# rebots-online/InstantIR

Hardware: AMD Instinct MI355X
Metric: denoising steps/sec at 1024x1024 (InstantIR step: previewer UNet + LCM + Aggregator + UNet, CFG) (higher is better)
Workload: dtype f16 (fp32 accumulate); 1 GPU; BASELINE configs[1]: 1024x1024, batch 1/GPU, cfg 7.0 (2 rows), 30-step DDIM timetable, preview_start 0, full SDXL+TA-IP UNet x2 + Aggregator per step; images_per_gpu=1, weight_elements=4422072388, graph=True, finite=True, world=1

## Files before the change

### instantir_amd/csrc/gemm_conv.hip

```cpp
#include "common.h"
#include "gemm_geo.h"
#include "../../include/instantir_hip.h"
#include <stdlib.h>
#include <type_traits>

namespace {

using iir::Geo;

constexpr int BK = 64;
#define IIR_PIN() __builtin_amdgcn_sched_barrier(0)
constexpr int PF_TOUCHES = 4;

constexpr int gn_par(int bm, bool lw) { return lw && bm == 128 ? 2 : 1; }
constexpr int ring_bytes(int bm, int bn, int st, bool w8) { return st * (bm * 128 + (w8 ? bn * 64 : bn * 128)); }
constexpr int scratch_bytes(int waves_m, bool lw) { return 256 * waves_m * 2 * (lw ? 2 : 1); }
constexpr int lds_bytes(int bm, int bn, int st, int waves_m, bool w8, bool lw) { return ring_bytes(bm, bn, st, w8) + scratch_bytes(waves_m, lw) + bm * 8; }
constexpr int lnp_off(int bm, int bn) { return (bm * (2 * bn + 32) + 15) / 16 * 16; }
constexpr bool ln_out_fits(int bm, int bn, int st, bool w8) { return lnp_off(bm, bn) + bm * (bn / 8) * 8 <= ring_bytes(bm, bn, st, w8); }
constexpr bool gn_out_fits(int bm, int bn, int st, int nt, bool lw, bool w8 = false) {
    const int gnt = nt / gn_par(bm, lw);
    return bm % 64 == 0 && bn <= gnt && (long)lnp_off(bm, bn) + (long)gn_par(bm, lw) * (gnt / (bn / 8)) * bn * 8 <= ring_bytes(bm, bn, st, w8);
}

template <int N>
__device__ __forceinline__ void wait_vm_lgkm_and_barrier() {
    asm volatile("s_waitcnt vmcnt(%0) lgkmcnt(0)\n\ts_barrier" ::"n"(N) : "memory");
}

template <int N>
__device__ __forceinline__ void wait_vm_and_barrier() {
    asm volatile("s_waitcnt vmcnt(%0)\n\ts_barrier" ::"n"(N) : "memory");
}

template <typename E, int BM, int BN, int ST, bool CONV, int WAVES_M = 2, bool W8 = false, bool LW = false, bool F8 = false>
__global__ __launch_bounds__(128 * WAVES_M * (LW ? 2 : 1), (WAVES_M == 2 ? 2 : 1)) void gemm_kernel(const Geo g) {
    static_assert(!(F8 && (W8 || CONV)), "the all-fp8 build covers the linear layers; W8 is the fp16-activation form");
    static_assert(!(W8 && CONV), "the fp8-weight build covers the linear layers only");
    static_assert(!(LW && W8), "loader waves: fp16 / bf16 operands only");
    static_assert(ST >= 2 && ST <= 4, "ring depths the counted waits below cover");
    using E4 = typename ET<E>::x4;
    using E8 = typename ET<E>::x8;
    constexpr int NW = WAVES_M * 2;
    constexpr int NT = 64 * NW * (LW ? 2 : 1);
    constexpr int WM = BM / WAVES_M, WN = BN / 2;
    constexpr int MI = WM / 16, NI = WN / 16;
    constexpr int B_GROUPS = W8 ? BN / 16 : BN / 8;
    constexpr int A_INST = BM / 8 / NW, B_INST = (B_GROUPS + NW - 1) / NW;
    static_assert(W8 || B_GROUPS % NW == 0, "fp16 weight tile: every wave issues the same number of row groups");
    constexpr int B_STAGE_BYTES = W8 ? BN * 64 : BN * 128;
    constexpr int RING_BYTES = ring_bytes(BM, BN, ST, W8);
    extern __shared__ __attribute__((aligned(16))) char smem[];
    f16* As = (f16*)smem;
    f16* Bs = As + ST * BM * BK;
    constexpr int LOADS = A_INST + B_INST;
    constexpr int SCRATCH_BYTES = scratch_bytes(WAVES_M, LW);
    float2* rowstat = (float2*)(smem + RING_BYTES + SCRATCH_BYTES);
    constexpr int LNP_OFF = lnp_off(BM, BN);
    constexpr bool LN_OUT_FITS = ln_out_fits(BM, BN, ST, W8);
    constexpr int GN_PAR = gn_par(BM, LW), GN_NT = NT / GN_PAR;
    constexpr int GN_RG = GN_NT / (BN / 8);
    constexpr bool GN_OUT_FITS = gn_out_fits(BM, BN, ST, NT, LW, W8);

    const int tid = threadIdx.x;
    const int lane = tid & 63;
    const int wave_all = __builtin_amdgcn_readfirstlane(tid >> 6);
    const bool loader = LW && wave_all >= NW;
    const int wave = loader ? wave_all - NW : wave_all;
    const int wm = wave >> 1, wn = wave & 1;

    int tm, tn;
    if (!iir::tile_of_block(g, tm, tn)) return;
    const int m0 = tm * BM, n0 = tn * BN;

    const int srow = lane >> 3;
    const int schunk = (lane & 7) ^ srow;
    const f16* a_src[A_INST];
    int a_pix_y[A_INST], a_pix_x[A_INST];
    const f16* a_img[A_INST];
#pragma unroll
    for (int i = 0; i < A_INST; ++i) {
        int m = m0 + (i * NW + wave) * 8 + srow;
        if (m >= g.M) m = g.M - 1;
        if (!CONV) {
            a_src[i] = g.A + (long)m * g.lda + schunk * 8;
        } else {
            const int hw = g.Ho * g.Wo;
            const int img = m / hw, rem = m - img * hw;
            const int oy = rem / g.Wo, ox = rem - oy * g.Wo;
            a_img[i] = g.A + (long)img * g.x_img_stride + schunk * 8;
            a_pix_y[i] = oy * g.stride - g.pad;
            a_pix_x[i] = ox * g.stride - g.pad;
        }
    }
    const f16* b_src[B_INST];
#pragma unroll
    for (int i = 0; i < B_INST; ++i) {
        if (!W8) {
            int n = n0 + (i * NW + wave) * 8 + srow;
            if (n >= g.N) n = g.N - 1;
            b_src[i] = g.W + (long)n * g.K + schunk * 8;
        } else {
            const int r = (i * NW + wave) * 16 + (lane >> 2);
            int n = n0 + r;
            if (n >= g.N) n = g.N - 1;
            b_src[i] = (const f16*)((const char*)g.W + (long)n * g.K + (((lane & 3) ^ ((r >> 2) & 3)) * 16));
        }
    }

    const f16* cv_ptr[CONV ? A_INST : 1];
    int cv_inc[CONV ? A_INST : 1];
    int cv_c0 = 0, cv_tap = 0;
    auto conv_tap = [&](int tap) {
        const int ky = tap / g.ks, kx = tap - ky * g.ks;
#pragma unroll
        for (int i = 0; i < (CONV ? A_INST : 0); ++i) {
            const int iy = a_pix_y[i] + ky, ix = a_pix_x[i] + kx;
            bool ok;
            long pix;
// ... 60 lines not shown
        a_off[s] = (wm * WM + frow) * 128 + phys * 16;
        if (!W8) b_off[s] = (wn * WN + frow) * 128 + phys * 16;
        else b_off[s] = (wn * WN + frow) * 64 + ((((fq >> 1) + 2 * s) ^ ((frow >> 2) & 3)) * 16) + (fq & 1) * 8;
    }

    f32x4 acc[MI][NI];
#pragma unroll
    for (int i = 0; i < MI; ++i)
#pragma unroll
        for (int j = 0; j < NI; ++j) acc[i][j] = (f32x4){0.f, 0.f, 0.f, 0.f};

    const int nk = g.K / BK;
    if (!LW || loader) {
        if (CONV) conv_seek(0);
#pragma unroll
        for (int s = 0; s < ST - 1; ++s)
            if (s < nk) stage(s, s);
    }
    constexpr int MAXP = 8;
    float2 lnp_in[MAXP];
    const int ln_lt = LW ? tid - 64 * NW : tid;
    if (g.ln_in && ln_lt >= 0 && ln_lt < BM) {
        const int m = min(m0 + ln_lt, g.M - 1);
#pragma unroll
        for (int j = 0; j < MAXP; ++j)
            lnp_in[j] = ((const float2*)g.ln_in)[(long)min(j, g.ln_parts - 1) * g.M + m];

        float sm = 0.f;
#pragma unroll
        for (int j = 0; j < MAXP; ++j) sm += j < g.ln_parts ? lnp_in[j].x : 0.f;
        const float inv_p = 1.0f / (float)g.ln_parts, mean = sm * inv_p;
        float m2 = 0.f, dev = 0.f;
#pragma unroll
        for (int j = 0; j < MAXP; ++j) {
            const float d = lnp_in[j].x - mean;
            m2 += j < g.ln_parts ? lnp_in[j].y : 0.f;
            dev += j < g.ln_parts ? d * d : 0.f;
        }
        const float var = (m2 + (float)g.ln_part_cols * dev) * inv_p / (float)g.ln_part_cols;
        const float rstd = rsqrtf(var + g.ln_eps);
        rowstat[ln_lt] = make_float2(rstd, -rstd * mean);
        }

    using BF = std::conditional_t<W8, long, E8>;
    auto frags = [&](int buf, int s, E8 (&af)[MI], BF (&bf)[NI]) {
        const char* as = (const char*)(As + buf * BM * BK);
        const char* bs = (const char*)Bs + buf * B_STAGE_BYTES;
#pragma unroll
        for (int i = 0; i < MI; ++i) af[i] = *(const E8*)(as + a_off[s] + i * 16 * 128);
#pragma unroll
        for (int j = 0; j < NI; ++j) bf[j] = *(const BF*)(bs + b_off[s] + j * 16 * (W8 ? 64 : 128));
    };
    auto mma = [&](const E8 (&af)[MI], const BF (&bf)[NI]) {
        if constexpr (F8) {
#pragma unroll
            for (int i = 0; i < MI; ++i)
#pragma unroll
                for (int j = 0; j < NI; ++j)
                    acc[i][j] = iir::mfma16_f8x2(bf[j], af[i], acc[i][j]);
        } else if constexpr (!W8) {
#pragma unroll
            for (int i = 0; i < MI; ++i)
#pragma unroll
                for (int j = 0; j < NI; ++j)
                    acc[i][j] = ET<E>::mfma16(bf[j], af[i], acc[i][j]);
        } else {
            long a8[MI];
#pragma unroll
            for (int i = 0; i < MI; ++i) a8[i] = iir_fp8x8(af[i]);
#pragma unroll
            for (int i = 0; i < MI; ++i)
#pragma unroll
                for (int j = 0; j < NI; ++j)
                    acc[i][j] = __builtin_amdgcn_mfma_f32_16x16x32_fp8_fp8(bf[j], a8[i], acc[i][j], 0, 0, 0);
        }
    };
    auto admit = [&](int tiles_after) {
        if (ST >= 4 && tiles_after >= 2) wait_vm_lgkm_and_barrier<(ST >= 4 ? 2 * LOADS : 0)>();
        else if (ST >= 3 && tiles_after >= 1) wait_vm_lgkm_and_barrier<(ST >= 3 ? LOADS : 0)>();
        else wait_vm_lgkm_and_barrier<0>();
    };
    f32x4 pre_c1[NI];
    E4 pre_c0[NI];
    auto preload_cols = [&]() {
#pragma unroll
        for (int j = 0; j < NI; ++j) {
            const int nc = min(n0 + wn * WN + j * 16 + fq * 4, g.N - 4);
            pre_c1[j] = g.ln_in ? *(const f32x4*)(g.ln_colsum + nc) : (f32x4){0.f, 0.f, 0.f, 0.f};
            if (g.bias) pre_c0[j] = *(const E4*)((const E*)g.bias + nc);
            else for (int t = 0; t < 4; ++t) pre_c0[j][t] = (E)0.f;
        }
    };
    E8 a0[MI], a1[MI];
    BF b0[NI], b1[NI];
    auto admit2 = [&](int tiles_after) {
        __builtin_amdgcn_s_waitcnt(0xC07F);
        if (ST >= 4 && tiles_after >= 2) wait_vm_and_barrier<(ST >= 4 ? 2 * LOADS : 0)>();
        else if (ST >= 3 && tiles_after >= 1) wait_vm_and_barrier<(ST >= 3 ? LOADS : 0)>();
        else wait_vm_and_barrier<0>();
    };
    if constexpr (!LW) {
        {
            const int rem = nk - 1;
            admit(rem < ST - 2 ? rem : ST - 2);
            if (ST - 1 < nk) stage(ST - 1, ST - 1);
            frags(0, 0, a0, b0);
            IIR_PIN();
            frags(0, 1, a1, b1);
            IIR_PIN();
            mma(a0, b0);
        }
        int cur = 0;
        for (int kt = 1; kt < nk; ++kt) {
            const int rem = nk - 1 - kt;
            admit2(rem < ST - 2 ? rem : ST - 2);
            if (kt - 1 + ST < nk) stage(kt - 1 + ST, cur);
            cur = cur + 1 == ST ? 0 : cur + 1;
            frags(cur, 0, a0, b0);
            IIR_PIN();
            mma(a1, b1);
            frags(cur, 1, a1, b1);
            IIR_PIN();
            mma(a0, b0);
        }
        preload_cols();
        mma(a1, b1);
    } else if (loader) {
        {
            const int rem = nk - 1;
            admit(rem < ST - 2 ? rem : ST - 2);
            if (ST - 1 < nk) stage(ST - 1, ST - 1);
        }
        int cur = 0;
        for (int kt = 0; kt + 1 < nk; ++kt) {
            const int rem = nk - 2 - kt;
            admit(rem < ST - 2 ? rem : ST - 2);
            if (kt + ST < nk) stage(kt + ST, cur);
            cur = cur + 1 == ST ? 0 : cur + 1;
        }
    } else {
        admit(0);
        frags(0, 0, a0, b0);
        IIR_PIN();
        frags(0, 1, a1, b1);
        IIR_PIN();
        mma(a0, b0);
        int cur = 0;
        for (int kt = 1; kt < nk; ++kt) {
            admit2(0);
            cur = cur + 1 == ST ? 0 : cur + 1;
            frags(cur, 0, a0, b0);
            IIR_PIN();
            mma(a1, b1);
            frags(cur, 1, a1, b1);
            IIR_PIN();
            mma(a0, b0);
        }
        preload_cols();
        mma(a1, b1);
    }

    bool xdone = false;
    if constexpr (BM == 64 && BN == 128 && ST == 3 && !CONV && !W8 && !LW && WAVES_M == 2 && std::is_same<E, f16>::value) {
    if (g.xa_on) {
        constexpr int KROWS = 144, KIMG = KROWS * 128, VROW = 288, VIMG = 64 * VROW;
        static_assert(2 * KIMG + 2 * VIMG <= RING_BYTES, "K / V images of two heads must fit the idle ring");
        asm volatile("s_waitcnt lgkmcnt(0)\n\ts_barrier" ::: "memory");
        const int img = m0 / g.xa_tq, hd0 = n0 >> 6;
        char* kl = smem;
        char* vl = smem + 2 * KIMG;
        const int tk0 = g.xa_tk[0], tk1 = g.xa_tk[1];
        const int vch0 = (tk0 + 7) >> 3, vch1 = (tk1 + 7) >> 3;
#pragma unroll
        for (int it = 0; it < 9; ++it) {
            const int s = (it * 4 + wave) * 64 + lane, hh = s >= 1152 ? 1 : 0, sl = s - hh * 1152;
            const int row = sl >> 3, ch = (sl & 7) ^ (row & 7);
            const bool ip = row >= 80;
            const int key = ip ? min(row - 80, tk1 - 1) : min(row, tk0 - 1);
            const f16* src = (ip ? g.xa_k[1] + (long)img * g.xa_kb[1] + (long)key * g.xa_ldk[1]
                                 : g.xa_k[0] + (long)img * g.xa_kb[0] + (long)key * g.xa_ldk[0]) + (hd0 + hh) * 64 + ch * 8;
            glds16(src, kl + (it * 4 + wave) * 1024);
        }
#pragma unroll
        for (int it = 0; it < 9; ++it) {
            const int s = (it * 4 + wave) * 64 + lane, hh = s >= 1152 ? 1 : 0, sl = s - hh * 1152;
            const int d = sl / 18, c = sl - d * 18;
            const bool ip = c >= 10;
            const int cc = ip ? min(c - 10, vch1 - 1) : min(c, vch0 - 1);
            const long rowv = (long)((hd0 + hh) * 64 + d);
            const f16* src = (ip ? g.xa_vt[1] + rowv * g.xa_ldvt[1] + (long)img * g.xa_vb[1]
                                 : g.xa_vt[0] + rowv * g.xa_ldvt[0] + (long)img * g.xa_vb[0]) + cc * 8;
            glds16(src, vl + (it * 4 + wave) * 1024);
        }
        typedef E E4v __attribute__((ext_vector_type(4)));
        E8 qf[MI][2];
#pragma unroll
        for (int i = 0; i < MI; ++i) {
            const float2 rs = g.ln_in ? rowstat[wm * WM + i * 16 + frow] : make_float2(1.f, 0.f);
#pragma unroll
            for (int j = 0; j < NI; ++j)
#pragma unroll
                for (int t = 0; t < 4; ++t)
                    qf[i][j >> 1][(j & 1) * 4 + t] = (E)iir::epi_affine(acc[i][j][t], rs, pre_c1[j][t], (float)pre_c0[j][t]);
        }
        asm volatile("s_waitcnt vmcnt(0)\n\ts_barrier" ::: "memory");
        f32x4 sa[MI][9];
        const char* kh = kl + wn * KIMG;
#pragma unroll
        for (int kb = 0; kb < 9; ++kb) {
            const int kr = kb * 16 + frow;
            const char* krow = kh + kr * 128 + (fq & 1) * 8;
            E8 kf[2];
#pragma unroll
            for (int ks = 0; ks < 2; ++ks) {
                const E4v lo = *(const E4v*)(krow + (((4 * ks + (fq >> 1)) ^ (kr & 7)) << 4));
                const E4v hi = *(const E4v*)(krow + (((4 * ks + 2 + (fq >> 1)) ^ (kr & 7)) << 4));
                for (int t = 0; t < 4; ++t) { kf[ks][t] = lo[t]; kf[ks][4 + t] = hi[t]; }
            }
#pragma unroll
            for (int i = 0; i < MI; ++i) {
                f32x4 z = {0.f, 0.f, 0.f, 0.f};
                z = ET<E>::mfma16(kf[0], qf[i][0], z);
// ... 312 lines not shown
                            m2 += pj.y + d * d * (8.0f * (float)j / (float)(j + 1));
                        }
                        ((float2*)g.ln_out)[(long)tn * g.M + m0 + tid] = make_float2(mean, m2);
                    }
                }
            }
        } else {
            touch_next_weights();
#pragma unroll 1
            for (int c = tid; c < TOTAL; c += NT) {
                const int r = c / CPR, cc = c - r * CPR;
                const int m = m0 + r, n = no_tile + cc * 8;
                if (m >= g.M || n >= No) continue;
                long mc = m, mr = m;
                if (remap) {
                    const int hw = g.Ho * g.Wo, img = m / hw, rem = m - img * hw;
                    if (g.y_img_rows) mc = (long)img * g.y_img_rows + rem;
                    if (g.res_img_rows) mr = (long)img * g.res_img_rows + rem;
                }
                const E* tp = (const E*)(ct + r * cs + cc * 16);
#pragma unroll 1
                for (int t = 0; t < 8 && n + t < No; ++t) {
                    float v = (float)tp[t];
                    if (g.Ct && n + t >= g.tr_from) { ((E*)g.Ct)[(long)(n + t - g.tr_from) * g.ldct + mc] = (E)(v * g.out_scale); continue; }
                    if (use_res) v += (float)((const E*)g.res)[mr * g.ldr + n + t];
                    ((E*)g.C)[mc * g.ldc + n + t] = (E)(v * g.out_scale);
                }
            }
        }
    };
    if (paired) write_out(std::integral_constant<int, BN / 16>{});
    else write_out(std::integral_constant<int, BN / 8>{});
    asm volatile("s_waitcnt vmcnt(0)" ::: "memory");
}

template <typename E, int BM, int BN, int ST, bool CONV, int WAVES_M = 2, bool W8 = false, bool LW = false, bool F8 = false>
int launch_k(const Geo& g0, hipStream_t stream) {
    constexpr int NT = 128 * WAVES_M * (LW ? 2 : 1);
    constexpr size_t lds = lds_bytes(BM, BN, ST, WAVES_M, W8, LW);
    Geo g = g0;
    if (g.c_fp8) {
        if (CONV || g.M % BM || g.N % BN || g.ldc % 8 || (uintptr_t)g.C % 8 || g.Ct || g.c_f32 || g.ln_out || g.gn_out || g.res_img_rows || g.y_img_rows ||
            (g.res && !g.r_vec) || g.dtype != IIR_DT_F16) return IIR_EINVAL;
        g.c_vec = 1; g.st_wt = 0;
    }
    if (g.gn_out) {
        constexpr bool fits = gn_out_fits(BM, BN, ST, NT, LW, W8);
        if (!fits || g.epi != IIR_EPI_PLAIN || g.c_f32 || g.Ct || g.ln_out || g.M % BM || g.N % BN || !g.c_vec || (g.res && !g.r_vec) ||
            (CONV && (g.y_img_rows | g.res_img_rows)))
            return IIR_EINVAL;
    }
    if (g.ln_out) {
        constexpr bool fits = ln_out_fits(BM, BN, ST, W8);
        if (!fits || CONV || g.epi != IIR_EPI_PLAIN || g.c_f32 || g.Ct || g.M % BM || g.N % BN || !g.c_vec || (g.res && !g.r_vec))
            return IIR_EINVAL;
    }
    iir::xcd_partition(g, BM, BN, 3.0 * 1048576.);
    const dim3 grid(8 * g.rm * g.rn), block(NT);
    const auto kern = gemm_kernel<E, BM, BN, ST, CONV, WAVES_M, W8, LW, F8>;
    static unsigned long long lds_set = 0;
    if (!iir_ensure_dynamic_lds((const void*)kern, lds, lds_set)) return IIR_ELAUNCH;
    iir_launch(kern, grid, block, lds, stream, g);
    return iir_launch_status();
}

template <int BM, int BN, int ST, int WAVES_M = 2, bool LW = false>
int launch(const Geo& g, bool conv, hipStream_t stream) {
    constexpr bool T5_3 = BM == 64 && BN == 160 && ST == 3 && WAVES_M == 2;
    constexpr bool FP8_TILE = T5_3 || (ST == 2 && WAVES_M == 2 && !LW);
    if (g.f8 || g.wscale) {
        if (conv || g.dtype != IIR_DT_F16) return IIR_EINVAL;
        if constexpr (FP8_TILE) {
            if (g.f8) return launch_k<f16, BM, BN, ST, false, WAVES_M, false, LW, true>(g, stream);
            if constexpr (!LW) return launch_k<f16, BM, BN, ST, false, WAVES_M, true>(g, stream);
        }
        return IIR_EINVAL;
    }
    if (g.dtype == IIR_DT_BF16) {
        if constexpr (ST == 2 && WAVES_M == 2 && !LW)
            return conv ? launch_k<bf16, BM, BN, ST, true>(g, stream) : launch_k<bf16, BM, BN, ST, false>(g, stream);
        return IIR_EINVAL;
    }
    if (!conv) return launch_k<f16, BM, BN, ST, false, WAVES_M, false, LW>(g, stream);
    if constexpr (!LW || ST == 3) return launch_k<f16, BM, BN, ST, true, WAVES_M, false, LW>(g, stream);
    return IIR_EINVAL;
}

struct TileShape { int bm, bn; };
constexpr TileShape kTiles[] = {{0, 0}, {128, 128}, {128, 64}, {64, 64}, {128, 160}, {64, 160}, {256, 128}};
constexpr int N_TILES = sizeof(kTiles) / sizeof(kTiles[0]) - 1;

constexpr int ONE_PER_CU_MIN_K = 1280;

int pick_tile(int M, int N, bool paired, int K = 0) {
    if (K >= ONE_PER_CU_MIN_K && (long)((M + 63) / 64) * ((N + 159) / 160) <= 256) return 5;
    long best = -1;
    int pick = 1;
    for (int t = 1; t <= 5; ++t) {
        const long blocks = (long)((M + kTiles[t].bm - 1) / kTiles[t].bm) * ((N + kTiles[t].bn - 1) / kTiles[t].bn);
        const long cost = ((blocks + 511) / 512) * 2 * (kTiles[t].bm + kTiles[t].bn);
        if (best < 0 || cost < best || (cost == best && kTiles[t].bm * kTiles[t].bn > kTiles[pick].bm * kTiles[pick].bn)) {
            best = cost;
            pick = t;
        }
    }
    return pick;
}

struct Resolved { int id, bm, bn, st, nt; bool lw; };

Resolved resolve_tile(int M, int N, int K, bool conv, int dtype, bool wscale, bool f8, int tile) {
    const bool f16 = dtype == IIR_DT_F16;
    if (tile < 0 || tile > N_TILES) return {-1, 0, 0, 0, 0, false};
    if (tile == 0) {
        static const bool t4_lw = !(getenv("IIR_T4_LW") && atoi(getenv("IIR_T4_LW")) == 0);
        if (t4_lw && f16 && !wscale && !f8 && K >= ONE_PER_CU_MIN_K && M % 128 == 0 && N % 160 == 0 &&
            (long)(M / 128) * (N / 160) <= 256 && (long)(M / 64) * (N / 160) > 256 && pick_tile(M, N, false, K) == 5)
            return {54, 128, 160, 3, 512, true};
        tile = pick_tile(M, N, false, K);
    }
    const int bm = kTiles[tile].bm, bn = kTiles[tile].bn;
    const long blocks = (long)((M + bm - 1) / bm) * ((N + bn - 1) / bn);
    const bool one_per_cu = tile == 5 && blocks <= 256 && K >= ONE_PER_CU_MIN_K && f16;
    if (one_per_cu && (!wscale || f8)) return {55, bm, bn, 3, 512, true};
    const int stages = one_per_cu ? 3 : 2;
    return {tile + 10 * stages, bm, bn, stages, tile == 6 ? 512 : 256, false};
}

bool gemm8_auto(const Geo& g, bool conv) {
    return !conv && (g.f8 ? 2 * g.K : g.K) >= 640 && (long)(g.M / 256) * (g.N / 320) >= 256 && iir::gemm8_covers(g, 320);
}

int dispatch(const Geo& g, bool conv, int tile, hipStream_t stream) {
    if (g.xa_on) return conv ? IIR_EINVAL : launch<64, 128, 3>(g, false, stream);
    if (tile == 0 && gemm8_auto(g, conv)) return iir::gemm8_launch(g, 320, stream);
    if (tile == 91 || tile == 92) return conv ? IIR_EINVAL : iir::gemm8_launch(g, tile == 91 ? 320 : 256, stream);
    if (tile < 10) tile = resolve_tile(g.M, g.N, g.f8 ? 2 * g.K : g.K, conv, g.dtype, g.wscale != nullptr, g.f8 != 0, tile).id;
    switch (tile) {
        case 21: return launch<128, 128, 2>(g, conv, stream);
        case 31: return launch<128, 128, 3>(g, conv, stream);
        case 22: return launch<128, 64, 2>(g, conv, stream);
        case 23: return launch<64, 64, 2>(g, conv, stream);
        case 24: return launch<128, 160, 2>(g, conv, stream);
        case 34: return launch<128, 160, 3>(g, conv, stream);
        case 25: return launch<64, 160, 2>(g, conv, stream);
        case 35: return launch<64, 160, 3>(g, conv, stream);
        case 54: return launch<128, 160, 3, 2, true>(g, conv, stream);
        case 55: return launch<64, 160, 3, 2, true>(g, conv, stream);
        case 65: return launch<64, 160, 4, 2, true>(g, conv, stream);
        case 75: return launch<64, 160, 2, 2, true>(g, conv, stream);
        case 26: return launch<256, 128, 2, 4>(g, conv, stream);
        case 36: return launch<256, 128, 3, 4>(g, conv, stream);
        case 90:
            if (g.epi == IIR_EPI_PLAIN) return IIR_EINVAL;
            return launch<256, 320, 2, 4>(g, conv, stream);
        default: return IIR_EINVAL;
    }
}

void finish_geo(Geo& g) {
    g.st_wt = (long)g.M * g.ldc * 2 < (1L << 31);
    if (g.pf_lines <= 0) { g.pf = (const char*)g.W; g.pf_lines = 1; }
    g.c_vec = (g.ldc % 8 == 0) && ((uintptr_t)g.C % 16 == 0);
    g.r_vec = g.res && (g.ldr % 8 == 0) && ((uintptr_t)g.res % 16 == 0);
}

}

extern "C" int iir_gemm_tile_bn(int32_t tile) { tile %= 10; return (tile >= 1 && tile <= N_TILES) ? kTiles[tile].bn : -1; }

extern "C" int iir_gemm_pick_tile(int32_t M, int32_t N, int32_t K, int32_t paired) { return pick_tile(M, N, paired != 0, K); }

extern "C" int iir_gemm_ln_parts(int32_t M, int32_t N, int32_t K) {
    if (M <= 0 || N <= 0 || K <= 0) return 0;
    const Resolved r = resolve_tile(M, N, K, false, IIR_DT_F16, false, false, 0);
    if (M % r.bm || N % r.bn || N / r.bn > 8) return 0;
    return N / r.bn;
}

static int fill_gemm_geo(const iir_gemm_desc* d, Geo& g);

extern "C" int iir_gemm_gn_supported(int32_t M, int32_t N, int32_t K, int32_t is_conv) {
    if (M <= 0 || N <= 0 || K <= 0 || M % 64) return 0;
    const Resolved r = resolve_tile(M, N, K, is_conv != 0, IIR_DT_F16, false, false, 0);
    if (M % r.bm || N % r.bn) return 0;
    return gn_out_fits(r.bm, r.bn, r.st, r.nt, r.lw) ? 1 : 0;
}

extern "C" int iir_gemm_fp8_out_supported(int32_t M, int32_t N, int32_t K, int32_t paired) {
    if (M <= 0 || N <= 0 || K <= 0 || K % 128) return 0;
    (void)paired;
    const Resolved r = resolve_tile(M, N, K, false, IIR_DT_F16, true, true, 0);
    return (M % r.bm == 0 && N % r.bn == 0) ? 1 : 0;
}

extern "C" int iir_gemm_f16(const iir_gemm_desc* d, void* stream) {
    (void)hipGetLastError();
    Geo g{};
    const int rc = fill_gemm_geo(d, g);
    if (rc != IIR_OK) return rc;
    return dispatch(g, false, d->tile, (hipStream_t)stream);
}

extern "C" int iir_gemm_resolve_tile(const iir_gemm_desc* d) {
    Geo g{};
    if (fill_gemm_geo(d, g) != IIR_OK) return -1;
    if (g.xa_on) return 93;
    if (d->tile != 0) return d->tile;
    if (gemm8_auto(g, false)) return 91;
    return resolve_tile(g.M, g.N, g.f8 ? 2 * g.K : g.K, false, g.dtype, g.wscale != nullptr, g.f8 != 0, 0).id;
}

static int fill_gemm_geo(const iir_gemm_desc* d, Geo& g) {
    if (!d || !d->A || !d->W || !d->C) return IIR_EINVAL;
    if (d->M <= 0 || d->N <= 0 || d->K <= 0 || d->K % BK) return IIR_EINVAL;
    if (d->N % 4 || d->lda % 8 || d->ldc % 4) return IIR_EINVAL;
    if (d->epi != IIR_EPI_PLAIN && (d->N % 16)) return IIR_EINVAL;
    if (d->epi == IIR_EPI_SFT && !d->res) return IIR_EINVAL;
    if (d->rowbias && d->rows_per_rb <= 0) return IIR_EINVAL;
    if (d->epi < IIR_EPI_PLAIN || d->epi > IIR_EPI_XATTN) return IIR_EINVAL;
    if (d->epi == IIR_EPI_XATTN) {
        const iir_attn_kv* kv = d->xattn_kv;
        if (!kv || d->dtype != IIR_DT_F16 || d->N % 128 || d->M % 64 || d->xattn_tq <= 0 || d->xattn_tq % 64 || d->M % d->xattn_tq) return IIR_EINVAL;
        if (d->res || d->rowbias || d->act || d->Ct || d->c_f32 || d->wscale || d->ln_stats_out || d->gn_stats_out) return IIR_EINVAL;
        if (d->ldc % 8 || (uintptr_t)d->C % 16 || (d->tile != 0 && d->tile != 93)) return IIR_EINVAL;
        if (kv[0].Tkv < 1 || kv[0].Tkv > 80 || kv[1].Tkv < 1 || kv[1].Tkv > 64) return IIR_EINVAL;
        for (int sgm = 0; sgm < 2; ++sgm) {
            if (!kv[sgm].K || !kv[sgm].Vt || (uintptr_t)kv[sgm].K % 16 || (uintptr_t)kv[sgm].Vt % 16) return IIR_EINVAL;
            if (kv[sgm].ldk % 8 || kv[sgm].k_batch_stride % 8 || kv[sgm].ldvt % 8 || kv[sgm].vt_batch_stride % 8) return IIR_EINVAL;
            g.xa_k[sgm] = (const f16*)kv[sgm].K; g.xa_ldk[sgm] = kv[sgm].ldk; g.xa_kb[sgm] = kv[sgm].k_batch_stride;
            g.xa_vt[sgm] = (const f16*)kv[sgm].Vt; g.xa_ldvt[sgm] = kv[sgm].ldvt; g.xa_vb[sgm] = kv[sgm].vt_batch_stride;
            g.xa_tk[sgm] = kv[sgm].Tkv;
        }
        g.xa_on = 1; g.xa_tq = d->xattn_tq;
    }
    g.A = (const f16*)d->A; g.lda = d->lda; g.W = (const f16*)d->W; g.C = (f16*)d->C; g.ldc = d->ldc;
    g.M = d->M; g.N = d->N; g.K = d->K;
    g.bias = (const f16*)d->bias; g.rowbias = (const f16*)d->rowbias; g.ldrb = d->ldrb; g.rows_per_rb = d->rows_per_rb;
    g.res = (const f16*)d->res; g.ldr = d->ldr; g.epi = d->epi == IIR_EPI_XATTN ? IIR_EPI_PLAIN : d->epi; g.act = d->act;
    g.out_scale = d->out_scale == 0.f ? 1.f : d->out_scale;
    g.pf = (const char*)d->prefetch; g.pf_lines = d->prefetch ? (int)(d->prefetch_bytes / 128) : 0;
    finish_geo(g);
    if (d->dtype != IIR_DT_F16 && d->dtype != IIR_DT_BF16) return IIR_EINVAL;
    g.dtype = d->dtype;
    if (d->c_f32) {
        if (d->epi != IIR_EPI_PLAIN || d->bias || d->rowbias || d->res || d->Ct || d->act || d->ldc % 4 || (uintptr_t)d->C % 16) return IIR_EINVAL;
        g.c_f32 = 1;
    }
    if (d->wscale) {
        if (d->c_f32 || d->K % 64 || (uintptr_t)d->W % 16 || (uintptr_t)d->wscale % 16 || d->dtype != IIR_DT_F16) return IIR_EINVAL;
        g.wscale = (const float*)d->wscale;
    }
    if (d->c_fp8) {
        if (d->epi == IIR_EPI_XATTN || d->epi == IIR_EPI_SFT || d->c_f32 || d->Ct || d->ln_stats_out || d->gn_stats_out || d->dtype != IIR_DT_F16) return IIR_EINVAL;
        g.c_fp8 = 1;
    }
    g.a_scale = 1.f;
    if (d->a_fp8) {
        if (!d->wscale || d->K % 128 || d->lda % 16 || (uintptr_t)d->A % 16 || d->ln_stats_in || d->epi == IIR_EPI_XATTN) return IIR_EINVAL;
        g.f8 = 1;
        g.a_scale = d->a_scale == 0.f ? 1.f : d->a_scale;
        g.K = d->K / 2; g.lda = d->lda / 2;
    }
    if (d->Ct) {
        if (d->epi != IIR_EPI_PLAIN || d->tr_from < 0 || d->tr_from >= d->N || d->tr_from % 8 || d->ldct < d->M) return IIR_EINVAL;
        g.Ct = (f16*)d->Ct; g.ldct = d->ldct; g.tr_from = d->tr_from;
        g.ct_vec = (d->ldct % 8 == 0) && ((uintptr_t)d->Ct % 16 == 0);
    }
    if (d->ln_stats_out) {
        if ((uintptr_t)d->ln_stats_out % 8 || d->c_f32 || d->Ct || d->epi != IIR_EPI_PLAIN) return IIR_EINVAL;
        g.ln_out = (float*)d->ln_stats_out;
    }
    if (d->gn_stats_out) {
        if ((uintptr_t)d->gn_stats_out % 8 || d->M % 64 || d->epi != IIR_EPI_PLAIN || d->c_f32 || d->Ct || d->ln_stats_out || d->wscale) return IIR_EINVAL;
        g.gn_out = (float*)d->gn_stats_out;
    }
    if (d->ln_stats_in) {
        if (!d->ln_colsum || d->ln_parts <= 0 || d->ln_parts > 8 || d->ln_part_cols <= 0 || (long)d->ln_parts * d->ln_part_cols != d->K || d->c_f32 ||
            (uintptr_t)d->ln_stats_in % 8 || (uintptr_t)d->ln_colsum % 16 || !(d->ln_eps > 0.f)) return IIR_EINVAL;
        g.ln_in = (const float*)d->ln_stats_in; g.ln_colsum = (const float*)d->ln_colsum;
        g.ln_parts = d->ln_parts; g.ln_part_cols = d->ln_part_cols; g.ln_eps = d->ln_eps;
    }
    return IIR_OK;
}

extern "C" int iir_conv2d_nhwc_f16(const iir_conv_desc* c, void* stream) {
    (void)hipGetLastError();
    if (!c || !c->X || !c->Wt || !c->Y || !c->zero_page) return IIR_EINVAL;
    if (c->ksize != 3 && c->ksize != 1) return IIR_EINVAL;
    if (c->Cin % BK || c->ldx % 8 || c->Cout % 4 || c->ldy % 4) return IIR_EINVAL;
    if (c->stride != 1 && c->stride != 2) return IIR_EINVAL;
    if (c->upsample && c->stride != 1) return IIR_EINVAL;
// ... 29 lines not shown
```

### instantir_amd/ops.py

```python
from __future__ import annotations

import ctypes as C

import torch

from . import lib as L
from .lib import ACT_GELU, ACT_NONE, ACT_QUICKGELU, ACT_SILU, EPI_GEGLU, EPI_PLAIN, EPI_SFT, EPI_XATTN


def _stream():
    return torch.cuda.current_stream().cuda_stream


def _p(t):
    return None if t is None else t.data_ptr()


_DT = {torch.float16: 0, torch.bfloat16: 1}


def _chk2d(t, name, dtype=torch.float16):
    if t.dtype != dtype or t.dim() != 2 or t.stride(1) != 1 or not t.is_cuda:
        raise ValueError(f"{name}: expected a 2-D {dtype} CUDA tensor with unit column stride, got {t.dtype} {tuple(t.shape)} {t.stride()}")


class LaunchProfiler:

    def __init__(self):
        self.records = []
        self._pool = []

    def events(self):
        h = L.load()
        e0, e1 = h.iir_timing_event_create(), h.iir_timing_event_create()
        if not e0 or not e1:
            raise L.HipLibraryError("hipEventCreate failed")
        self._pool += [e0, e1]
        return e0, e1

    def summary(self):
        torch.cuda.synchronize()
        h = L.load()
        out = {}
        us = C.c_float()
        for cls, flops, e0, e1, nbytes in self.records:
            L.check(h.iir_timing_elapsed_us(e0, e1, C.byref(us)), "iir_timing_elapsed_us")
            d = out.setdefault(cls, {"launches": 0, "ms": 0.0, "flops": 0.0, "bytes": 0.0})
            d["launches"] += 1
            d["ms"] += us.value * 1e-3
            d["flops"] += flops
            d["bytes"] += nbytes
        for e in self._pool:
            h.iir_timing_event_destroy(e)
        self._pool = []
        return out


PROFILER = None

_TILE_NAMES = {1: "128x128", 2: "128x64", 3: "64x64", 4: "128x160", 5: "64x160", 6: "256x128", 0: "256x320"}


def auto_tile(M, N, paired=False, K=0):
    return L.load().iir_gemm_pick_tile(M, N, K, int(paired))


class _Timed:
    def __init__(self, cls, flops, nbytes=0.0):
        self.cls, self.flops, self.nbytes = cls, flops, nbytes

    def __enter__(self):
        if PROFILER is not None:
            e0, e1 = PROFILER.events()
            L.check(L.load().iir_timing_arm(e0, e1), "iir_timing_arm")
            PROFILER.records.append((self.cls, self.flops, e0, e1, self.nbytes))

    def __exit__(self, *a):
        pass


_zero_pages = {}


def zero_page(device):
    z = _zero_pages.get(device)
    if z is None:
        z = torch.zeros(256, dtype=torch.float16, device=device)
        _zero_pages[device] = z
    return z


FP8_MAX = 448.0


class Fp8Weight:

    def __init__(self, q, scale):
        self.q, self.scale = q, scale
        self.shape = q.shape

    def numel(self):
        return self.q.numel() // 2

    def data_ptr(self):
        return self.q.data_ptr()


def quantize_fp8_rows(w):
    w32 = w.float()
    scale = (w32.abs().amax(dim=1).clamp_min(1e-12) / FP8_MAX).contiguous()
    q = (w32 / scale[:, None]).clamp(-FP8_MAX, FP8_MAX).to(torch.float8_e4m3fn).contiguous()
    return q, scale


_FP8_DTYPES = (torch.float8_e4m3fn, torch.uint8)


def gemm_fp8(a8, w8, out, a_scale=1.0, bias=None, res=None, epi=EPI_PLAIN, act=ACT_NONE, tile=0, prefetch=None, out_t=None):
    if not isinstance(w8, Fp8Weight):
        raise ValueError("gemm_fp8: w8 must be an Fp8Weight")
    if a8.dtype not in _FP8_DTYPES or a8.dim() != 2 or a8.stride(1) != 1 or not a8.is_cuda:
        raise ValueError("gemm_fp8: a8 must be a 2-D CUDA view of torch.float8_e4m3fn (or its bytes) with contiguous rows")
    M, K = a8.shape
    N = w8.q.shape[0]
    if w8.q.shape[1] != K or K % 128 or a8.stride(0) % 16:
        raise ValueError("gemm_fp8: K must match, K % 128 == 0, row stride % 16 == 0")
    dt = torch.float16
    c_fp8 = out.dtype in _FP8_DTYPES
    if c_fp8:
        if out.dim() != 2 or out.stride(1) != 1 or out.stride(0) % 8 or not out.is_cuda:
            raise ValueError("gemm_fp8: an fp8 `out` needs contiguous rows with a stride % 8 == 0")
    else:
        _chk2d(out, "out", dt)
    n_out = (N if epi == EPI_PLAIN else N // 2) if out_t is None else out_t[1]
    if out.shape != (M, n_out):
        raise ValueError(f"out shape {tuple(out.shape)} != {(M, n_out)}")
    for t_, n_ in ((bias, "bias"), (res, "res")):
        if t_ is not None and t_.dtype != dt:
            raise ValueError(f"{n_}: fp16 expected")
    d = L.GemmDesc()
    d.c_fp8 = int(c_fp8)
    if out_t is not None:
        _fill_out_t(d, out_t, dt, M, N, c_fp8, "out_t: fp16 (N - tr_from, M), with an fp16 `out`")
# ... 85 lines not shown
        raise ValueError(msg)
    d.Ct, d.ldct, d.tr_from = ct.data_ptr(), ct.stride(0), tr_from


def _fill_kv(table, kv):
    for i, (k, k_rows, vt, vbs, tkv) in enumerate(kv):
        _chk2d(k, "k"); _chk2d(vt, "vt")
        e = table[i]
        e.K, e.ldk, e.k_batch_stride = k.data_ptr(), k.stride(0), k_rows * k.stride(0)
        e.Vt, e.ldvt, e.vt_batch_stride = vt.data_ptr(), vt.stride(0), vbs
        e.Tkv = tkv


def gemm(a, w, out, bias=None, rowbias=None, rows_per_rb=1, res=None, epi=EPI_PLAIN, act=ACT_NONE, out_scale=1.0,
         tile=0, prefetch=None, out_t=None, wscale=None, ln_out=None, ln_in=None, gn_out=None, xattn=None):
    dt = a.dtype
    if isinstance(w, Fp8Weight):
        w, wscale = w.q, w.scale
    if wscale is not None:
        if w.dtype not in (torch.float8_e4m3fn, torch.uint8) or w.dim() != 2 or not w.is_contiguous() or not w.is_cuda:
            raise ValueError("fp8 weights: contiguous 2-D CUDA tensor of torch.float8_e4m3fn (or its bytes)")
        if wscale.dtype != torch.float32 or wscale.numel() != w.shape[0] or not wscale.is_contiguous():
            raise ValueError("wscale: contiguous fp32 (N,)")
        if dt != torch.float16:
            raise ValueError("fp8 weights take fp16 activations")
    if dt not in _DT:
        raise ValueError(f"a: fp16 or bf16 expected, got {dt}")
    c_f32 = out.dtype == torch.float32
    _chk2d(a, "a", dt); _chk2d(out, "out", torch.float32 if c_f32 else dt)
    if wscale is None:
        _chk2d(w, "w", dt)
    for t_, n_ in ((bias, "bias"), (rowbias, "rowbias"), (res, "res")):
        if t_ is not None and t_.dtype != dt:
            raise ValueError(f"{n_}: dtype {t_.dtype} does not match the operands ({dt})")
    M, K = a.shape
    N = w.shape[0]
    if w.shape[1] != K or not w.is_contiguous():
        raise ValueError("w must be contiguous (N,K) with K matching a")
    n_out = (N if epi in (EPI_PLAIN, EPI_XATTN) else N // 2) if out_t is None else out_t[1]
    if out.shape != (M, n_out):
        raise ValueError(f"out shape {tuple(out.shape)} != {(M, n_out)}")
    d = L.GemmDesc()
    d.A, d.lda = a.data_ptr(), a.stride(0)
    d.W = w.data_ptr()
    d.C, d.ldc = out.data_ptr(), out.stride(0)
    d.M, d.N, d.K = M, N, K
    d.bias = _p(bias)
    _fill_operands(d, dt, M, N, rowbias, rows_per_rb, res, prefetch, gn_out)
    d.epi, d.act, d.out_scale, d.tile = epi, act, out_scale, tile
    d.dtype, d.c_f32 = _DT[dt], int(c_f32)
    if wscale is not None:
        d.wscale = wscale.data_ptr()
    if ln_out is not None:
        if ln_out.dtype != torch.float32 or not ln_out.is_contiguous() or ln_out.dim() != 3 or ln_out.shape[1:] != (M, 2) \
                or ln_out.shape[0] != ln_parts(M, N, K) or tile != 0:
            raise ValueError("ln_out: contiguous fp32 (ln_parts(M, N, K), M, 2), tile = 0")
        d.ln_stats_out = ln_out.data_ptr()
    if ln_in is not None:
        part, colsum, eps = ln_in
        if part.dtype != torch.float32 or not part.is_contiguous() or part.dim() != 3 or part.shape[1:] != (M, 2) or K % part.shape[0]:
            raise ValueError("ln_in partials: contiguous fp32 (parts, M, 2) with parts dividing K")
        if colsum.dtype != torch.float32 or colsum.numel() != N or not colsum.is_contiguous():
            raise ValueError("ln_in colsum: contiguous fp32 (N,)")
        d.ln_stats_in, d.ln_colsum, d.ln_parts, d.ln_part_cols, d.ln_eps = part.data_ptr(), colsum.data_ptr(), part.shape[0], K // part.shape[0], eps
    kv_keep = None
    if (epi == EPI_XATTN) != (xattn is not None):
        raise ValueError("epi = EPI_XATTN goes with xattn = (kv, Tq)")
    if xattn is not None:
        kvs, tq = xattn
        if len(kvs) != 2:
            raise ValueError("xattn: two K / V^T segments (text, IP tokens)")
        kv_keep = (L.AttnKV * 2)()
        _fill_kv(kv_keep, kvs)
        d.xattn_kv, d.xattn_tq = kv_keep, tq
    if xattn is not None:
        tile = 93
    elif tile == 0:
        tile = auto_tile(M, N, epi != EPI_PLAIN, K)
    if out_t is not None:
        _fill_out_t(d, out_t, dt, M, N, False, "out_t must hold (N - tr_from, M)")
    No = N // 2 if epi not in (EPI_PLAIN, EPI_XATTN) else N
    if xattn is not None:
        cls = "gemm_kernel<64x128,gemm+xattn>"
    elif PROFILER is not None and d.tile == 0 and L.load().iir_gemm_resolve_tile(C.byref(d)) == 91:
        cls = "gemm8_kernel<256x320,gemm>"
    else:
        cls = "gemm_kernel<%s,%s>" % (_TILE_NAMES[tile % 10], "gemm" if wscale is None else "gemm-w8")
    xa_flops = 4.0 * M * N * sum(k[4] for k in xattn[0]) if xattn is not None else 0.0
    with _Timed(cls, 2.0 * M * N * K + xa_flops,
                2.0 * (M * K + N * K * (1.0 if wscale is None else 0.5) + M * No + (M * No if res is not None else 0))):
        L.check(L.load().iir_gemm_f16(C.byref(d), _stream()), "iir_gemm_f16")
    return out


def conv2d(x, w, out, ksize=3, stride=1, upsample=False, bias=None, rowbias=None, rows_per_rb=1, res=None,
           epi=EPI_PLAIN, act=ACT_NONE, out_scale=1.0, tile=0, y_img_rows=0, res_img_rows=0, pad_mode=0, prefetch=None, gn_out=None):
    R, H, Wd, Cin = x.shape
    dt = x.dtype
    if dt not in _DT or x.stride(3) != 1 or x.stride(1) != Wd * x.stride(2):
        raise ValueError("x must be an NHWC fp16 / bf16 view with dense rows (pixel and image strides are free)")
    _chk2d(out, "out", dt)
    for t_, n_ in ((w, "w"), (bias, "bias"), (rowbias, "rowbias"), (res, "res")):
        if t_ is not None and t_.dtype != dt:
            raise ValueError(f"{n_}: dtype {t_.dtype} does not match x ({dt})")
    Cout = w.shape[0]
    if tuple(w.shape[1:]) != (ksize, ksize, Cin) or not w.is_contiguous():
        raise ValueError("w must be contiguous (Cout,k,k,Cin)")
    d = L.ConvDesc()
    d.X, d.ldx = x.data_ptr(), x.stride(2)
    d.R, d.H, d.Wd, d.Cin = R, H, Wd, Cin
    d.Wt = w.data_ptr()
    d.Y, d.ldy = out.data_ptr(), out.stride(0)
    d.Cout, d.ksize, d.stride, d.upsample = Cout, ksize, stride, int(bool(upsample))
    d.bias = _p(bias)
    d.dtype = _DT[dt]
    Hi, Wi = (2 * H, 2 * Wd) if upsample else (H, Wd)
    pad2 = 1 if pad_mode == 1 else 2 * (ksize // 2)
    Mo = R * ((Hi + pad2 - ksize) // stride + 1) * ((Wi + pad2 - ksize) // stride + 1)
    _fill_operands(d, dt, Mo, Cout, rowbias, rows_per_rb, res, prefetch, gn_out)
    d.epi, d.act, d.out_scale, d.tile = epi, act, out_scale, tile
    if tile == 0:
        Kc = ksize * ksize * Cin
        tile = auto_tile(Mo, Cout, epi != EPI_PLAIN, Kc)
    d.zero_page = zero_page(x.device).data_ptr()
    d.x_img_stride, d.y_img_rows, d.res_img_rows, d.pad_mode = x.stride(0), y_img_rows, res_img_rows, pad_mode
    Co = Cout // 2 if epi != EPI_PLAIN else Cout
    with _Timed("gemm_kernel<%s,conv>" % _TILE_NAMES[tile % 10], 2.0 * Mo * Cout * ksize * ksize * Cin,
                2.0 * (R * H * Wd * Cin + Cout * ksize * ksize * Cin + Mo * Co + (Mo * Co if res is not None else 0))):
        L.check(L.load().iir_conv2d_nhwc_f16(C.byref(d), _stream()), "iir_conv2d_nhwc_f16")
    return out


ATTN_LOG2E = 1.4426950408889634


def attn_q_factor(scale=0.125):
    import numpy as np
    return float(np.float32(scale) * np.float32(ATTN_LOG2E))


def attention(q, o, kv, batch, heads, Tq, scale=0.125, causal=False, q_prescaled=False, head_dim=64, ident_from=0):
    _chk2d(q, "q")
    d = L.AttnDesc()
    if o.dtype in _FP8_DTYPES:
        if o.dim() != 2 or o.stride(1) != 1 or o.stride(0) % 4 or not o.is_cuda:
            raise ValueError("attention: an fp8 `o` needs contiguous rows with a stride % 4 == 0")
        d.o_fp8 = 1
    else:
        _chk2d(o, "o")
    d.Q, d.ldq, d.q_batch_stride = q.data_ptr(), q.stride(0), Tq * q.stride(0)
    d.O, d.ldo, d.o_batch_stride = o.data_ptr(), o.stride(0), Tq * o.stride(0)
    d.batch, d.heads, d.Tq, d.nseg, d.scale = batch, heads, Tq, len(kv), scale
    d.causal = int(bool(causal))
    d.q_prescaled = int(bool(q_prescaled))
    _fill_kv(d.kv, kv)
    if ident_from:
        if head_dim != 64:
            raise ValueError("attention: identity rows need head_dim 64")
        with _Timed("attn_kernel", 4.0 * ident_from * heads * Tq * head_dim * kv[0][4],
                    2.0 * ident_from * heads * head_dim * (2 * Tq + 2 * kv[0][4]) + 4.0 * (batch - ident_from) * heads * Tq * head_dim):
            L.check(L.load().iir_attention_d64_ident_f16(C.byref(d), int(ident_from), _stream()), "iir_attention_d64_ident_f16")
        return o
    with _Timed("attn_kernel", 4.0 * batch * heads * Tq * head_dim * sum(k[4] for k in kv),
                2.0 * batch * heads * head_dim * (2 * Tq + 2 * sum(k[4] for k in kv))):
        if head_dim == 64:
            L.check(L.load().iir_attention_d64_f16(C.byref(d), _stream()), "iir_attention_d64_f16")
        else:
            L.check(L.load().iir_attention_f16(C.byref(d), head_dim, _stream()), "iir_attention_f16")
    return o

# ... 384 lines not shown
```

Baseline: 17.40 steps/s.

## Route large-K plain GEMMs to a 256x256 one-per-CU kernel and add a 128x256 loader-wave tile

Adds a dispatch rule that sends plain, bias-free, non-residual linear GEMMs with large K and roughly one tile per CU to the existing 8-wave gemm kernel at a 256x256 tile. It also adds a new 128x256 loader-wave tile variant whose main loop splits the N fragments into two groups to limit register pressure, and relaxes that variant's launch bounds to one wave per SIMD. The aim is to fill all CUs exactly once for QKV-like projections and cut wave-quantization tail waste. The new 128x256 tile is only reachable by explicit tile id, so its register and occupancy tradeoff only matters if it gets picked. The profiler labeling in Python is updated to match.

```diff
diff --git a/instantir_amd/csrc/gemm_conv.hip b/instantir_amd/csrc/gemm_conv.hip
--- a/instantir_amd/csrc/gemm_conv.hip
+++ b/instantir_amd/csrc/gemm_conv.hip
@@ -33,8 +33,10 @@
     asm volatile("s_waitcnt vmcnt(%0)\n\ts_barrier" ::"n"(N) : "memory");
 }
 
+constexpr bool split_n_tile(int bm, int bn, bool lw) { return lw && bm == 128 && bn == 256; }
+constexpr int min_waves_per_simd(int bm, int bn, int waves_m, bool lw) { return waves_m == 2 && !split_n_tile(bm, bn, lw) ? 2 : 1; }
 template <typename E, int BM, int BN, int ST, bool CONV, int WAVES_M = 2, bool W8 = false, bool LW = false, bool F8 = false>
-__global__ __launch_bounds__(128 * WAVES_M * (LW ? 2 : 1), (WAVES_M == 2 ? 2 : 1)) void gemm_kernel(const Geo g) {
+__global__ __launch_bounds__(128 * WAVES_M * (LW ? 2 : 1), min_waves_per_simd(BM, BN, WAVES_M, LW)) void gemm_kernel(const Geo g) {
     static_assert(!(F8 && (W8 || CONV)), "the all-fp8 build covers the linear layers; W8 is the fp16-activation form");
     static_assert(!(W8 && CONV), "the fp8-weight build covers the linear layers only");
     static_assert(!(LW && W8), "loader waves: fp16 / bf16 operands only");
@@ -261,14 +263,15 @@
     };
     f32x4 pre_c1[NI];
     E4 pre_c0[NI];
+    auto preload_col = [&](int j) {
+        const int nc = min(n0 + wn * WN + j * 16 + fq * 4, g.N - 4);
+        pre_c1[j] = g.ln_in ? *(const f32x4*)(g.ln_colsum + nc) : (f32x4){0.f, 0.f, 0.f, 0.f};
+        if (g.bias) pre_c0[j] = *(const E4*)((const E*)g.bias + nc);
+        else for (int t = 0; t < 4; ++t) pre_c0[j][t] = (E)0.f;
+    };
     auto preload_cols = [&]() {
 #pragma unroll
-        for (int j = 0; j < NI; ++j) {
-            const int nc = min(n0 + wn * WN + j * 16 + fq * 4, g.N - 4);
-            pre_c1[j] = g.ln_in ? *(const f32x4*)(g.ln_colsum + nc) : (f32x4){0.f, 0.f, 0.f, 0.f};
-            if (g.bias) pre_c0[j] = *(const E4*)((const E*)g.bias + nc);
-            else for (int t = 0; t < 4; ++t) pre_c0[j][t] = (E)0.f;
-        }
+        for (int j = 0; j < NI; ++j) preload_col(j);
     };
     E8 a0[MI], a1[MI];
     BF b0[NI], b1[NI];
@@ -317,6 +320,64 @@
             if (kt + ST < nk) stage(kt + ST, cur);
             cur = cur + 1 == ST ? 0 : cur + 1;
         }
+    } else if constexpr (split_n_tile(BM, BN, LW)) {
+        static_assert(!W8 && !F8 && NI % 2 == 0, "fp16 / bf16 operands");
+        constexpr int NG = NI / 2;
+        E8 bg0[NG], bg1[NG];
+        auto frags_a = [&](int buf, int s, E8 (&af)[MI]) {
+            const char* as = (const char*)(As + buf * BM * BK);
+#pragma unroll
+            for (int i = 0; i < MI; ++i) af[i] = *(const E8*)(as + a_off[s] + i * 16 * 128);
+        };
+        auto frags_b = [&](int buf, int s, int grp, E8 (&bf)[NG]) {
+            const char* bs = (const char*)Bs + buf * B_STAGE_BYTES;
+#pragma unroll
+            for (int j = 0; j < NG; ++j) bf[j] = *(const E8*)(bs + b_off[s] + (grp * NG + j) * 16 * 128);
+        };
+        auto mma_g = [&](const E8 (&af)[MI], const E8 (&bf)[NG], auto grp_tag) {
+            constexpr int GRP = decltype(grp_tag)::value;
+#pragma unroll
+            for (int i = 0; i < MI; ++i)
+#pragma unroll
+                for (int j = 0; j < NG; ++j)
+                    acc[i][GRP * NG + j] = ET<E>::mfma16(bf[j], af[i], acc[i][GRP * NG + j]);
+        };
+        constexpr std::integral_constant<int, 0> G0{};
+        constexpr std::integral_constant<int, 1> G1{};
+        admit(0);
+        frags_a(0, 0, a0); frags_b(0, 0, 0, bg0);
+        IIR_PIN();
+        frags_b(0, 0, 1, bg1);
+        IIR_PIN();
+        mma_g(a0, bg0, G0);
+        frags_a(0, 1, a1); frags_b(0, 1, 0, bg0);
+        IIR_PIN();
+        mma_g(a0, bg1, G1);
+        frags_b(0, 1, 1, bg1);
+        IIR_PIN();
+        mma_g(a1, bg0, G0);
+        int cur = 0;
+        for (int kt = 1; kt < nk; ++kt) {
+            admit2(0);
+            cur = cur + 1 == ST ? 0 : cur + 1;
+            frags_a(cur, 0, a0); frags_b(cur, 0, 0, bg0);
+            IIR_PIN();
+            mma_g(a1, bg1, G1);
+            frags_b(cur, 0, 1, bg1);
+            IIR_PIN();
+            mma_g(a0, bg0, G0);
+            frags_a(cur, 1, a1); frags_b(cur, 1, 0, bg0);
+            IIR_PIN();
+            mma_g(a0, bg1, G1);
+            frags_b(cur, 1, 1, bg1);
+            IIR_PIN();
+            mma_g(a1, bg0, G0);
+        }
+#pragma unroll
+        for (int j = 0; j < NG; ++j) preload_col(j);
+        mma_g(a1, bg1, G1);
+#pragma unroll
+        for (int j = NG; j < NI; ++j) preload_col(j);
     } else {
         admit(0);
         frags(0, 0, a0, b0);
@@ -795,12 +856,12 @@
         return IIR_EINVAL;
     }
     if (!conv) return launch_k<f16, BM, BN, ST, false, WAVES_M, false, LW>(g, stream);
-    if constexpr (!LW || ST == 3) return launch_k<f16, BM, BN, ST, true, WAVES_M, false, LW>(g, stream);
+    if constexpr ((!LW || ST == 3) && !split_n_tile(BM, BN, LW)) return launch_k<f16, BM, BN, ST, true, WAVES_M, false, LW>(g, stream);
     return IIR_EINVAL;
 }
 
 struct TileShape { int bm, bn; };
-constexpr TileShape kTiles[] = {{0, 0}, {128, 128}, {128, 64}, {64, 64}, {128, 160}, {64, 160}, {256, 128}};
+constexpr TileShape kTiles[] = {{0, 0}, {128, 128}, {128, 64}, {64, 64}, {128, 160}, {64, 160}, {256, 128}, {128, 256}};
 constexpr int N_TILES = sizeof(kTiles) / sizeof(kTiles[0]) - 1;
 
 constexpr int ONE_PER_CU_MIN_K = 1280;
@@ -844,9 +905,16 @@
     return !conv && (g.f8 ? 2 * g.K : g.K) >= 640 && (long)(g.M / 256) * (g.N / 320) >= 256 && iir::gemm8_covers(g, 320);
 }
 
+int qkv_one_per_cu(const Geo& g, bool conv) {
+    if (conv || !g.Ct || g.res || g.wscale || g.f8 || g.epi != IIR_EPI_PLAIN || g.K < ONE_PER_CU_MIN_K) return 0;
+    const long tiles = (long)(g.M / 256) * (g.N / 256);
+    return iir::gemm8_covers(g, 256) && tiles >= 224 && tiles <= 256 ? 92 : 0;
+}
+
 int dispatch(const Geo& g, bool conv, int tile, hipStream_t stream) {
     if (g.xa_on) return conv ? IIR_EINVAL : launch<64, 128, 3>(g, false, stream);
     if (tile == 0 && gemm8_auto(g, conv)) return iir::gemm8_launch(g, 320, stream);
+    if (tile == 0 && qkv_one_per_cu(g, conv)) tile = qkv_one_per_cu(g, conv);
     if (tile == 91 || tile == 92) return conv ? IIR_EINVAL : iir::gemm8_launch(g, tile == 91 ? 320 : 256, stream);
     if (tile < 10) tile = resolve_tile(g.M, g.N, g.f8 ? 2 * g.K : g.K, conv, g.dtype, g.wscale != nullptr, g.f8 != 0, tile).id;
     switch (tile) {
@@ -860,6 +928,7 @@
         case 35: return launch<64, 160, 3>(g, conv, stream);
         case 54: return launch<128, 160, 3, 2, true>(g, conv, stream);
         case 55: return launch<64, 160, 3, 2, true>(g, conv, stream);
+        case 57: return launch<128, 256, 3, 2, true>(g, conv, stream);
         case 65: return launch<64, 160, 4, 2, true>(g, conv, stream);
         case 75: return launch<64, 160, 2, 2, true>(g, conv, stream);
         case 26: return launch<256, 128, 2, 4>(g, conv, stream);
@@ -921,6 +990,7 @@
     if (g.xa_on) return 93;
     if (d->tile != 0) return d->tile;
     if (gemm8_auto(g, false)) return 91;
+    if (qkv_one_per_cu(g, false)) return qkv_one_per_cu(g, false);
     return resolve_tile(g.M, g.N, g.f8 ? 2 * g.K : g.K, false, g.dtype, g.wscale != nullptr, g.f8 != 0, 0).id;
 }
 
diff --git a/instantir_amd/ops.py b/instantir_amd/ops.py
--- a/instantir_amd/ops.py
+++ b/instantir_amd/ops.py
@@ -58,7 +58,7 @@
 
 PROFILER = None
 
-_TILE_NAMES = {1: "128x128", 2: "128x64", 3: "64x64", 4: "128x160", 5: "64x160", 6: "256x128", 0: "256x320"}
+_TILE_NAMES = {1: "128x128", 2: "128x64", 3: "64x64", 4: "128x160", 5: "64x160", 6: "256x128", 7: "128x256", 0: "256x320"}
 
 
 def auto_tile(M, N, paired=False, K=0):
@@ -310,10 +310,13 @@
     No = N // 2 if epi not in (EPI_PLAIN, EPI_XATTN) else N
     if xattn is not None:
         cls = "gemm_kernel<64x128,gemm+xattn>"
-    elif PROFILER is not None and d.tile == 0 and L.load().iir_gemm_resolve_tile(C.byref(d)) == 91:
-        cls = "gemm8_kernel<256x320,gemm>"
     else:
-        cls = "gemm_kernel<%s,%s>" % (_TILE_NAMES[tile % 10], "gemm" if wscale is None else "gemm-w8")
+        if PROFILER is not None and d.tile == 0:
+            tile = L.load().iir_gemm_resolve_tile(C.byref(d))
+        if tile in (91, 92):
+            cls = "gemm8_kernel<256x%d,gemm>" % (320 if tile == 91 else 256)
+        else:
+            cls = "gemm_kernel<%s,%s>" % (_TILE_NAMES[tile % 10], "gemm" if wscale is None else "gemm-w8")
     xa_flops = 4.0 * M * N * sum(k[4] for k in xattn[0]) if xattn is not None else 0.0
     with _Timed(cls, 2.0 * M * N * K + xa_flops,
                 2.0 * (M * K + N * K * (1.0 if wscale is None else 0.5) + M * No + (M * No if res is not None else 0))):
```

Measured after the change: 17.49 steps/s (median of 6 runs). Within noise of the previous version (+0.5%).
